# DJjjjhao/FIRA-ICSE

Measured on AMD Instinct MI355X. Metric: training commits/sec (FIRA default config), higher is better.
Workload: dtype f32; 1 GPU; BASELINE configs[1]: FIRA training step (fwd+bwd+Adam, dropout 0.1/0.2), batch 32 commits/GPU, fp32, 650-node graphs (mean nnz 1066/graph), vocab 24650; global_batch=32, parallelism=dp1

## Files before the change

### fira_icse_amd/_lib.py

```python
from __future__ import annotations

import ctypes as C
import os

HERE = os.path.dirname(os.path.abspath(__file__))
LIB_PATH = os.environ.get("FIRA_HIP_LIB") or os.path.join(HERE, "libfira_hip.so")


class FiraError(RuntimeError):
    pass


class Dims(C.Structure):
    _fields_ = [("sou_len", C.c_int32), ("sub_len", C.c_int32), ("ast_len", C.c_int32), ("tar_len", C.c_int32),
                ("d_model", C.c_int32), ("n_head", C.c_int32), ("n_layer", C.c_int32), ("vocab", C.c_int32),
                ("ast_vocab", C.c_int32), ("d_ff", C.c_int32)]


class Batch(C.Structure):
    _fields_ = [("B", C.c_int32), ("nnz", C.c_int32), ("sou", C.c_void_p), ("tar", C.c_void_p), ("mark", C.c_void_p),
                ("ast_change", C.c_void_p), ("tar_label", C.c_void_p), ("sub_token", C.c_void_p),
                ("n_nodes", C.c_int32), ("node_rows", C.c_void_p), ("rowptr", C.c_void_p), ("col", C.c_void_p),
                ("val", C.c_void_p), ("n_code", C.c_int32), ("code_rows", C.c_void_p), ("code_mark", C.c_void_p),
                ("n_mem", C.c_int32), ("mem_rows", C.c_void_p), ("mem_dst", C.c_void_p), ("head_rows", C.c_void_p),
# ... 43 lines not shown
    "fira_linear_x3": (_I, [_P, _I, _I, _P, _I, _P, _P, _P, _I, _I]),
    "fira_linear_dgrad_x3": (_I, [_P, _I, _I, _P, _I, _P, _P, _I, _I, _I]),
    "fira_dgrad_x3_splitk_planes_bytes": (_Z, [_I]),
    "fira_dgrad_x3_splitk": (_I, [_P, _I, _I, _P, _I, _P, _P, _P, _I, _I]),
    "fira_head_logits_x3_scratch_bytes": (_Z, [_I]),
    "fira_head_logits_x3": (_I, [_P, _I, _I, _P, _I, _P, _P, _P, _I, _P]),
    "fira_combination_block_fwd": (_I, [_P, _I, _P, _P, _P, _P, _P, _P, _P, _I, _P, _P, _P, _P, _P, _P, _P, _P, _P, _F, _U64, _U32, _U32, _I]),
    "fira_combination_block_bwd": (_I, [_P, _I, _P, _P, _P, _P, _P, _P, _P, _P, _P, _I, _P, _P, _P, _P, _P, _P, _I, _P, _F, _U64, _U32, _U32, _I]),
    "fira_combination_block_bwd_part_floats": (_I, []),
    "fira_embed_gather_fwd": (_I, [_P, _I, _I, _P, _P, _P, _P, _I, _I]),
    "fira_embed_gather_bwd": (_I, [_P, _I, _I, _P, _P, _P, _I, _I, _I]),
    "fira_combination_fwd": (_I, [_P, _I, _P, _P, _P, _P, _F, _U64, _U32]),
    "fira_combination_bwd": (_I, [_P, _I, _P, _P, _P, _P, _P, _P, _F, _U64, _U32]),
    "fira_add_layernorm_fwd": (_I, [_P, _I, _P, _P, _P, _P, _P, _P, _F, _U64, _U32]),
    "fira_linear_presum_f32": (_I, [_P, _I, _I, _P, _I, _P, _P, _P, _P, _F, _U64, _U32]),
    "fira_ln_linear_f32": (_I, [_P, _I, _I, _P, _I, _P, _P, _P, _I, _I, _P, _P, _P, _P]),
    "fira_ln_bwd_linear_f32": (_I, [_P, _I, _I, _P, _P, _P, _P, _P, _P, _P, _P, _P, _P, _P, _P, _F, _U64, _U32]),
    "fira_linear_layernorm_bf16_fwd": (_I, [_P, _I, _P, _I, _P, _I, _P, _P, _P, _P, _P, _P, _P, _F, _U64, _U32]),
    "fira_add_layernorm_bwd": (_I, [_P, _I, _P, _P, _P, _P, _P, _P, _P, _P, _F, _U64, _U32]),
    "fira_dropout_mask": (_I, [_P, _U64, _U32, _L, _F, _P]),
    "fira_colsum_f32": (_I, [_P, _I, _I, _P, _I, _P]),
    "fira_attention_fwd": (_I, [_P, _I, _I, _I, _I, _P, _I, _P, _I, _P, _I, _P, _I, _I, _P, _I]),
    "fira_attention_bwd": (_I, [_P, _I, _I, _I, _I, _P, _I, _P, _I, _P, _I, _P, _I, _I, _P, _I, _P, _I,
                                _P, _I, _P, _I, _P, _I]),
    "fira_attention_fwd_ex": (_I, [_P, _I, _I, _I, _I, _P, _I, _P, _I, _P, _I, _P, _I, _I, _P, _I, _P, _I, _I, _P]),
    "fira_attention_bwd_ex": (_I, [_P, _I, _I, _I, _I, _P, _I, _P, _I, _P, _I, _P, _I, _I, _P, _I, _P, _I,
                                   _P, _I, _P, _I, _P, _I, _P, _I, _I, _P]),
    "fira_decode_attention": (_I, [_P, _I, _I, _I, _P, _I, _P, _I, _P, _I, _P, _P, _I, _I, _I, _I, _P, _P, _I, _P, _P, _P]),
    "fira_copy_score_fwd": (_I, [_P, _I, _I, _I, _P, _P, _P, _P, _P]),
    "fira_copy_score_bwd": (_I, [_P, _I, _I, _I, _P, _P, _P, _P, _P, _P, _P, _P]),
    "fira_head_loss": (_I, [_P, _I, _I, _I, _I, _P, _P, _I, _P, _P, _P, _P, _P, _P, _P, _I]),
    "fira_adam_step": (_I, [_P, _L, _P, _P, _P, _P, _F, _F, _F, _F, _I, _P]),
    "fira_adam_step_mb": (_I, [_P, _L, _P, _P, _P, _P, _P, _F, _F, _F, _F, _I, _P, _P]),
    "fira_inv_count": (_I, [_P, _P, _P]),
    "fira_adam_step_count": (_I, [_P, _L, _P, _P, _P, _P, _F, _F, _F, _F, _I, _P]),
    "fira_pack_stats": (_I, [_P, _P, _P, _P]),
    "fira_debug_chain": (_I, [_P, _I, _I, _P]),
    "fira_train_fwd_bwd": (_I, [_P, _DP, _BP, _P, _P, _P, _Z, _OP, _P, _P, _P]),
    "fira_train_step": (_I, [_P, _DP, _BP, _P, _P, _P, _Z, _OP, _P, _P, C.POINTER(AdamOpts)]),
    "fira_gemm_wgrad_panel": (_I, [_P, _I, _I, _I, _I, _P, _I, _P, _I, _P, _I, _P, _P, _Z]),
    "fira_ffn_fwd": (_I, [_P, _I, _I] + [_P] * 11 + [_F, _U64, _U32, _I]),
    "fira_ffn_bwd": (_I, [_P, _I, _I] + [_P] * 17 + [_F, _U64, _U32, _I]),
    "fira_head_topk": (_I, [_P, _I, _I, _I, _P, _P, _P, _P, _I, _P, _P, _I]),
    "fira_train_step_rows": (_I, [_P, _DP, _BP, _P, _P, _P, _Z, _OP, _P, _P, C.POINTER(AdamOpts), _P]),
    "fira_adam_rows_sync": (_I, [_P, _DP, _P, C.POINTER(AdamOpts), _P]),
    "fira_adam_rows_catchup": (_I, [_P, _DP, _P, C.POINTER(AdamOpts), _P, _I, _P, _I]),
    "fira_adam_rows_step": (_I, [_P, _DP, _P, _P, C.POINTER(AdamOpts), _P, _P, _P, _I]),
    "fira_train_step_begin_rows": (_I, [_P, _DP, _BP, _P, _P, _P, _Z, _OP, _P, _P, _P, C.POINTER(AdamOpts), _P]),
    "fira_train_step_end_rows": (_I, [_P, _P, C.POINTER(AdamOpts), _P, _P, _P]),
    "fira_grad_sqsum_scratch_bytes": (_Z, []),
    "fira_grad_sqsum": (_I, [_P, _L, _P, _P, _I, _P]),
    "fira_clip_finish": (_I, [_P, _P, _I, _P, _P, _F]),
    "fira_adam_step_clip": (_I, [_P, _L, _P, _P, _P, _P, _F, _F, _F, _F, _I, _P, _P, _P]),
    "fira_adam_rows_step_clip": (_I, [_P, _DP, _P, _P, C.POINTER(AdamOpts), _P, _P, _P, _I, _P]),
    "fira_train_step_clip": (_I, [_P, _DP, _BP, _P, _P, _P, _Z, _OP, _P, _P, C.POINTER(AdamOpts), _P, _F, _P, _P]),
    "fira_train_step_begin": (_I, [_P, _DP, _BP, _P, _P, _P, _Z, _OP, _P, _P, _P]),
    "fira_train_step_end": (_I, [_P, _P, C.POINTER(AdamOpts), _P, _P]),
    "fira_f32_to_bf16": (_I, [_P, _L, _P, _P]),
    "fira_bf16_to_f32": (_I, [_P, _L, _P, _P]),
    "fira_prof_enable": (None, [_I]),
    "fira_prof_report": (_I, [_I, C.POINTER(C.c_double), C.POINTER(C.c_double), C.POINTER(C.c_double), C.POINTER(_L)]),
    "fira_param_groups": (_I, [_DP, C.POINTER(_L), C.POINTER(_L)]),
    "fira_host_node_lists": (_I, [_I, _I, _I, _I, _I] + [_P] * 7 + [_I] + [_P] * 14),
    "fira_host_collate_csr": (_I, [_I, _I, _P, _L, _P, _P, _P, _P, _P, _P, _P]),
    "fira_forward_dev": (_I, [_P, _DP, _BP, _P, _P, _Z, _P, _P, _P, _I]),
    "fira_decode_begin": (_I, [_P, _DP, _BP, _P, _P, _Z, _I]),
# ... 94 lines not shown
```

### fira_icse_amd/csrc/copyhead.hip

```cpp
#include "engine.h"
#include "adam_rows.h"
#include <stdlib.h>
#include "epilogue.h"
#include "decode_row.h"

namespace fira {

constexpr int T_MAX = 32;

__device__ __forceinline__ float tanh_fast(float x) {
    const float e = __expf(2.0f * x);
    return 1.0f - __fdividef(2.0f, 1.0f + e);
}

__global__ __launch_bounds__(256) void copy_score_fwd_kernel(int T, int S, const float* __restrict__ src,
                                                             const float* __restrict__ tgt,
                                                             const float* __restrict__ w,
                                                             const float* __restrict__ bias,
                                                             float* __restrict__ score, int qpk,
                                                             const int32_t* __restrict__ mem_valid, int slots,
                                                             const int32_t* __restrict__ tar_label, int V,
                                                             const int32_t* __restrict__ t_off) {
    __shared__ __attribute__((aligned(16))) float sm_tgt[T_MAX * FIRA_D];
    __shared__ unsigned sm_mask;
// ... 777 lines not shown
}
int head_loss(hipStream_t s, int BT, int T, int V, int S, const int32_t* compact_row, float* logits, int ldl,
              float* score, const int32_t* mem_valid, float* gate_logits, const int32_t* tar_label, float* loss_sum,
              int32_t* n_tok, int32_t* argmax_out, int want_grad, const int32_t* row_bt) {
    ProfScope prof(s, PROF_HEAD, 0.0);
    if (BT <= 0) return 0;
    const bool reg = (V % 2 == 0) && (V / 2 <= 256 * HL_PAIRS) && (ldl % 2 == 0) && ((uintptr_t)logits % 8 == 0);
    if (reg && !argmax_out)
        hipLaunchKernelGGL(head_loss_train_kernel, dim3(BT), dim3(256), 0, s, T, V, S, compact_row, logits, ldl, score,
                           mem_valid, gate_logits, tar_label, loss_sum, n_tok, want_grad, row_bt);
    else if (reg)
        hipLaunchKernelGGL(head_loss_kernel<true>, dim3(BT), dim3(256), 0, s, T, V, S, compact_row, logits, ldl, score,
                           mem_valid, gate_logits, tar_label, loss_sum, n_tok, argmax_out, want_grad, row_bt);
    else
        hipLaunchKernelGGL(head_loss_kernel<false>, dim3(BT), dim3(256), 0, s, T, V, S, compact_row, logits, ldl, score,
                           mem_valid, gate_logits, tar_label, loss_sum, n_tok, argmax_out, want_grad, row_bt);
    FIRA_CHECK_LAUNCH("head_loss");
    return 0;
}
int adam_step(hipStream_t s, int64_t n, float* p, const float* g, float* m, float* v, float lr, float beta1,
              float beta2, float eps, int step, const float* scale_ptr, int scale_is_count) {
    ProfScope prof(s, PROF_ADAM, 0.0);
    if (n <= 0) return 0;
    FIRA_REQUIRE(step >= 1, "adam_step: step must start at 1");
    const double bc1 = 1.0 - pow((double)beta1, step);
    const double bc2 = 1.0 - pow((double)beta2, step);
    const int grid = (int)std::min<int64_t>(cdiv64(n, 256), 256 * 16);
    hipLaunchKernelGGL(adam_kernel, dim3(grid), dim3(256), 0, s, n, p, g, m, v, lr, beta1, beta2, eps, (float)bc1,
                       (float)sqrt(bc2), scale_ptr, scale_is_count);
    FIRA_CHECK_LAUNCH("adam_step");
    return 0;
}
int adam_step_mb(hipStream_t s, int64_t n, float* p, const float* g0, const float* g1, float* m, float* v, float lr,
                 float beta1, float beta2, float eps, int step, const int32_t* n0, const int32_t* n1) {
    ProfScope prof(s, PROF_ADAM, 0.0);
    if (n <= 0) return 0;
    const double bc1 = 1.0 - pow((double)beta1, step);
    const double bc2 = 1.0 - pow((double)beta2, step);
    const int grid = (int)std::min<int64_t>(cdiv64(n, 256), 256 * 16);
    hipLaunchKernelGGL(adam_mb_kernel, dim3(grid), dim3(256), 0, s, n, p, g0, g1, m, v, lr, beta1, beta2, eps, (float)bc1,
                       (float)sqrt(bc2), n0, n1);
    FIRA_CHECK_LAUNCH("adam_step_mb");
    return 0;
}
AdamRowsHist adam_rows_hist(float beta1, float beta2, int end) {
    AdamRowsHist h;
    for (int k = 0; k < ADAM_ROWS_K; ++k) h.bc1[k] = h.bc2s[k] = 1.f;
    for (int j = std::max(1, end - ADAM_ROWS_K + 1); j <= end; ++j) {
        h.bc1[j % ADAM_ROWS_K] = (float)(1.0 - pow((double)beta1, j));
        h.bc2s[j % ADAM_ROWS_K] = (float)sqrt(1.0 - pow((double)beta2, j));
    }
    return h;
}
AdamRowsView adam_rows_view(const AdamRowsTables& tb, int table, float lr, float beta1, float beta2, float eps, int to) {
    AdamRowsView vw;
    if (to < 1) return vw;
    vw.m = tb.m + tb.off[table]; vw.v = tb.v + tb.off[table];
    vw.last = tb.last + (table ? tb.rows[0] : 0);
    vw.to = to; vw.lr = lr; vw.beta1 = beta1; vw.beta2 = beta2; vw.eps = eps; vw.gz = 0.f;
    vw.h = adam_rows_hist(beta1, beta2, to);
    return vw;
}
int adam_rows_step(hipStream_t s, const AdamRowsTables& tb, const float* g, float lr, float beta1, float beta2, float eps,
                   int step, const int32_t* n0, const float* count, int tables) {
    ProfScope prof(s, PROF_ADAM, 0.0);
    FIRA_REQUIRE(step >= 1 && tb.last && (n0 || count), "adam_rows_step: bad argument");
    const int it_lo = (tables & 1) ? 0 : tb.rows[0], it_hi = (tables & 2) ? tb.rows[0] + tb.rows[1] : tb.rows[0];
    const int total = it_hi - it_lo;
    if (total <= 0) return 0;
    const int grid = std::min(cdiv(total, 16), 256 * 8);
    hipLaunchKernelGGL(adam_rows_kernel, dim3(grid), dim3(256), 0, s, tb, g, lr, beta1, beta2, eps, step,
                       adam_rows_hist(beta1, beta2, step), n0, count, step % ADAM_ROWS_K == 0 ? 1 : 0, 0.0f, it_lo, it_hi);
// ... 13 lines not shown
    hipLaunchKernelGGL(adam_rows_catchup_kernel, dim3(grid), dim3(256), 0, s, tb, l, lr, beta1, beta2, eps, to,
                       adam_rows_hist(beta1, beta2, to), 0.0f);
    FIRA_CHECK_LAUNCH("adam_rows_catchup");
    return 0;
}
int inv_count(hipStream_t s, const int32_t* n_tok, float* out) {
    hipLaunchKernelGGL(inv_count_kernel, dim3(1), dim3(1), 0, s, n_tok, out);
    FIRA_CHECK_LAUNCH("inv_count");
    return 0;
}

}

extern "C" {
int fira_copy_score_fwd(void* stream, int B, int T, int S, const float* src, const float* tgt, const float* w,
                        const float* bias, float* score) {
    return fira::copy_score_fwd((hipStream_t)stream, B, T, S, src, tgt, w, bias, score);
}
int fira_copy_score_bwd(void* stream, int B, int T, int S, const float* src, const float* tgt, const float* w,
                        const float* dscore, float* dsrc, float* dtgt, float* dw, float* dbias) {
    return fira::copy_score_bwd((hipStream_t)stream, B, T, S, src, tgt, w, dscore, dsrc, dtgt, dw, dbias);
}
int fira_head_loss(void* stream, int BT, int T, int V, int S, const int32_t* compact_row, float* logits, int ldl,
                   float* score, const int32_t* mem_valid, float* gate_logits, const int32_t* tar_label,
                   float* loss_sum, int32_t* n_tok, int32_t* argmax_out, int want_grad) {
    return fira::head_loss((hipStream_t)stream, BT, T, V, S, compact_row, logits, ldl, score, mem_valid, gate_logits,
                           tar_label, loss_sum, n_tok, argmax_out, want_grad);
}
int fira_adam_step_mb(void* stream, int64_t n, float* p, const float* g0, const float* g1, float* m, float* v, float lr,
                      float beta1, float beta2, float eps, int step, const int32_t* n_tok0, const int32_t* n_tok1) {
    FIRA_REQUIRE(p && g0 && m && v && n_tok0 && step >= 1, "fira_adam_step_mb: bad argument");
    return fira::adam_step_mb((hipStream_t)stream, n, p, g0, g1, m, v, lr, beta1, beta2, eps, step, n_tok0, n_tok1);
}
int fira_inv_count(void* stream, const int32_t* n_tok, float* out) {
    return fira::inv_count((hipStream_t)stream, n_tok, out);
}
int fira_adam_step(void* stream, int64_t n, float* p, const float* g, float* m, float* v, float lr, float beta1,
                   float beta2, float eps, int step, const float* inv_scale_ntok) {
    return fira::adam_step((hipStream_t)stream, n, p, g, m, v, lr, beta1, beta2, eps, step, inv_scale_ntok, 0);
}
int fira_adam_step_count(void* stream, int64_t n, float* p, const float* g, float* m, float* v, float lr, float beta1,
                         float beta2, float eps, int step, const float* count) {
    FIRA_REQUIRE(p && g && m && v && count && step >= 1, "fira_adam_step_count: bad argument");
    return fira::adam_step((hipStream_t)stream, n, p, g, m, v, lr, beta1, beta2, eps, step, count, 1);
}
int fira_pack_stats(void* stream, const float* loss_sum, const int32_t* n_tok, float* out2) {
    FIRA_REQUIRE(loss_sum && n_tok && out2, "fira_pack_stats: null pointer argument");
    hipLaunchKernelGGL(fira::pack_stats_kernel, dim3(1), dim3(1), 0, (hipStream_t)stream, loss_sum, n_tok, out2);
    FIRA_CHECK_LAUNCH("pack_stats");
    return 0;
}
}
```

### fira_icse_amd/csrc/engine.h

```cpp
#pragma once
#include "common.h"
#include <string>
#include <vector>

namespace fira {

int gemm_f32(hipStream_t s, int tA, int tB, int M, int N, int K, const float* A, int lda, const float* B, int ldb,
             float* C, int ldc, const float* bias, int flags, int splitk);
int gemm_f32_ex(hipStream_t s, int tA, int tB, int M, int N, int K, const float* A, int lda, const float* B, int ldb,
                float* C, int ldc, const float* bias, int flags, int splitk, float* colsum,
                const int32_t* c_rows = nullptr, const float* relu_mask = nullptr);
int gemm_bf16_ex(hipStream_t s, int tA, int tB, int M, int N, int K, const float* A, int lda, const float* B, int ldb,
                 float* C, int ldc, const float* bias, int flags, int splitk, float* colsum,
                 const int32_t* c_rows = nullptr, const float* relu_mask = nullptr);
struct ShadowEntry { int64_t offset; int rows, cols, pitch_t; int64_t offset_t; };
constexpr int SHADOW_MAX = 64;
struct ShadowTable {
    int n = 0;
    int64_t wbt_elems = 0;
    int tile_start[SHADOW_MAX + 1] = {0};
    ShadowEntry e[SHADOW_MAX];
};
int weight_shadows(hipStream_t s, const ShadowTable& tab, const float* P, uint16_t* Wb, uint16_t* WbT);
int gemm_bf16_wb_ex(hipStream_t s, int M, int N, int K, const float* A, int lda, const uint16_t* Bb, int ldb, float* C,
// ... 176 lines not shown
                   const float* bias, float* score);
int copy_score_fwd_ex(hipStream_t s, int B, int T, int S, const float* src, const float* tgt, const float* w,
                      const float* bias, float* score, int qpk, const int32_t* mem_valid,
                      const int32_t* tar_label = nullptr, int V = 0,
                      const int32_t* t_off = nullptr);
int copy_score_bwd_ex(hipStream_t s, int B, int T, int S, const float* src, const float* tgt, const float* w,
                      const float* dscore, float* dsrc, float* dtgt, float* dw, float* dbias, const int32_t* mem_valid,
                      float* part = nullptr, const int32_t* t_off = nullptr);
int copy_score_bwd_blocks(int B, int S);
constexpr int COPY_PART_STRIDE = 264;
int decode_dist(hipStream_t s, int R, int V, int S, const float* logits, int ldl, const float* score,
                const int32_t* mem_valid, int qpk, const float* gate_logits, float* dist, int32_t* best_id,
                float* best_p, const float* x = nullptr, const float* wp = nullptr, const float* bp = nullptr);
int inv_count(hipStream_t s, const int32_t* n_tok, float* out);
int sample_dist(hipStream_t s, int R, int n_sample, int V, int S, const float* logits, int ldl, const float* score,
                const int32_t* mem_valid, const float* x, const float* wp, const float* bp, int T, int step,
                const int32_t* key, const uint64_t* seed_dev, float temperature, int top_k, float top_p, float* dist,
                int32_t* best_id, float* best_p);
int score_dist(hipStream_t s, int R, int n_cand, int V, int L, int S, const float* logits, int ldl, const float* score,
               const int32_t* mem_valid, const float* x, const float* wp, const float* bp, const int32_t* target,
               const int32_t* label, const int32_t* sou, const int32_t* sub, float* dist, float* p_word, float* p_entry,
               int32_t* entry, float* copy_share, float* p_label, int32_t* top_id, float* logp_word, float* logp_entry,
               float* logp_label);
int row_topk(hipStream_t s, int R, int V, int k, const float* logits, int ldl, int32_t* ids, float* vals);
int copy_score_bwd(hipStream_t s, int B, int T, int S, const float* src, const float* tgt, const float* w,
                   const float* dscore, float* dsrc, float* dtgt, float* dw, float* dbias);
int head_loss(hipStream_t s, int BT, int T, int V, int S, const int32_t* compact_row, float* logits, int ldl,
              float* score, const int32_t* mem_valid, float* gate_logits, const int32_t* tar_label, float* loss_sum,
              int32_t* n_tok, int32_t* argmax_out, int want_grad,
              const int32_t* row_bt = nullptr);
int adam_step(hipStream_t s, int64_t n, float* p, const float* g, float* m, float* v, float lr, float beta1,
              float beta2, float eps, int step, const float* scale_ptr, int scale_is_count = 0);
int adam_step_mb(hipStream_t s, int64_t n, float* p, const float* g0, const float* g1, float* m, float* v, float lr,
                 float beta1, float beta2, float eps, int step, const int32_t* n0, const int32_t* n1);
constexpr int ADAM_ROWS_K = 32;
struct AdamRowsHist { float bc1[ADAM_ROWS_K], bc2s[ADAM_ROWS_K]; };
struct AdamRowsTables { float *p, *m, *v; int64_t off[2]; int rows[2]; int32_t* last; };
struct AdamRowsView {
    const float *m = nullptr, *v = nullptr;
    const int32_t* last = nullptr;
    int to = 0;
    float lr = 0.f, beta1 = 0.f, beta2 = 0.f, eps = 0.f, gz = 0.f;
    AdamRowsHist h;
};
AdamRowsView adam_rows_view(const AdamRowsTables& tb, int table, float lr, float beta1, float beta2, float eps, int to);
struct AdamRowsLists { int n_lists; int end[4]; int table[4]; const int32_t* ids[4]; };
int adam_rows_step(hipStream_t s, const AdamRowsTables& tb, const float* g, float lr, float beta1, float beta2, float eps,
                   int step, const int32_t* n0, const float* count, int tables = 3);
int adam_rows_catchup(hipStream_t s, const AdamRowsTables& tb, const AdamRowsLists* ls, float lr, float beta1, float beta2,
                      float eps, int to);
AdamRowsHist adam_rows_hist(float beta1, float beta2, int end);
struct ClipClose {
    const int32_t* n_tok;
    const float* count;
    float max_norm;
    int n_slots;
};
size_t grad_sqsum_scratch_bytes();
int grad_sqsum(hipStream_t s, int64_t n, const float* g, fira_clip_state* st, int slot, void* scratch, const ClipClose* fin);
int clip_finish(hipStream_t s, fira_clip_state* st, const ClipClose& fin);
int adam_step_clip(hipStream_t s, int64_t n, float* p, const float* g, float* m, float* v, float lr, float beta1, float beta2,
                   float eps, int step, const int32_t* n0, const float* count, const fira_clip_state* st);
int adam_rows_step_clip(hipStream_t s, const AdamRowsTables& tb, const float* g, float lr, float beta1, float beta2, float eps,
                        int step, const int32_t* n0, const float* count, int tables, const fira_clip_state* st);

struct ParamInfo {
    std::string name;
// ... 25 lines not shown
```

### fira_icse_amd/csrc/engine.hip

```cpp
#include "engine.h"
#include <hip/hip_ext.h>
#include "epilogue.h"
#include <stdlib.h>
#include <map>
#include <mutex>

namespace fira {

static int64_t shadow_wbt_elems(const Layout& L);

struct Arena {
    char* base;
    size_t used = 0;
    explicit Arena(void* b) : base((char*)b) {}
    template <typename T>
    T* get(size_t n) {
        size_t bytes = (n * sizeof(T) + 255) / 256 * 256;
        T* p = base ? (T*)(base + used) : nullptr;
        used += bytes;
        return p;
    }
    float* f(size_t n) { return get<float>(n); }
};

// ... 969 lines not shown
    TRY(linear(s, R, p.V, D, dec_rows, D, c.P + L.wout, c.P + L.bout, p.logits, p.ldl));
    TRY(gemm_any(s, 0, 1, c.Td, D, D, dec, D, c.P + L.wt, D, p.tgt, D, nullptr, 0, 0, nullptr));
    if (c.deferred) TRY(main_wait(s, c.ev_src, __LINE__));
    TRY(copy_score_fwd_ex(s, p.B, p.T, Sm, p.src, p.tgt, c.P + L.wres, c.P + L.bres, p.score, 1, p.mem_valid,
                          argmax_out ? nullptr : c.bt->tar_label, p.V, c.dec_off));
    TRY(linear(s, c.Td, 2, D, dec, D, c.P + L.wp, c.P + L.bp, p.gate, 2));
    TRY(head_loss(s, c.Td, p.T, p.V, Sm, p.compact_row, p.logits, p.ldl, p.score, p.mem_valid, p.gate,
                  c.bt->tar_label, loss_sum, n_tok, argmax_out, want_grad, c.row_bt));
    return 0;
}

static inline int enc_wgrad_every(int n_rows, int n_layers) {
    static const int forced = [] { const char* e = getenv("FIRA_ENC_WGRAD_EVERY"); const int v = e ? atoi(e) : 0; return v >= 1 ? v : 0; }();
    if (forced) return forced;
    return n_rows <= 32768 ? std::max(1, n_layers) : 1;
}

static int group_a_final_stream(hipStream_t s, hipStream_t* out) {
    SideStream& sd = side();
    *out = s;
    if (sd.stream && sd.enabled) {
        TRY(aux_fork(s));
        hipEvent_t e2 = sd.ev();
        if (hipEventRecord(e2, sd.stream) != hipSuccess || hipStreamWaitEvent(sd.aux, e2, 0) != hipSuccess)
            return set_err("group-A mark: weight-gradient stream mark failed");
        *out = sd.aux;
    }
    return 0;
}

struct BwdMid {
    hipEvent_t ev_dmem = nullptr;
    hipEvent_t ev_groupA = nullptr;
};

static int backward_decoder(Ctx& c, int R, const int32_t* rows, hipEvent_t mid_event, BwdMid& mid) {
    Plan& p = *c.pl;
    const Layout& L = *c.L;
    hipStream_t s = c.s;
    const int D = FIRA_D, H = L.d.n_head, KV = p.nl * 2 * D, Sm = p.L + p.S;
    const fira_batch& bt = *c.bt;
    const int Nc = bt.n_nodes, Cc = bt.n_code, Mc = bt.n_mem;
    const float* dec = p.dec[p.nl - 1].x_f;
    float* G = c.G;

    gemm_group_reset();
    gemm_bf16_group_reset();
    gemm_wgrad_panel_reset();
    gemm_wgrad_panel_scratch(p.panel_scratch, p.panel_floats);
    red().reset(p.red_buf, p.red_cap);
    const bool so = side_on();
    hipStream_t ss = so ? side().aux : s;
    hipEvent_t ev_dfc = nullptr;
    if (c.ev_zero) TRY(main_wait(s, c.ev_zero, __LINE__));
    else TRY(zero(s, p.zero_beg, (size_t)((char*)p.zero_end - (char*)p.zero_beg)));
    if (R > 0) {
        if (so) TRY(aux_fork(s));
        if (c.wout_planes) TRY(dgrad_x3_splitk(ss, R, p.V, p.logits, p.ldl, p.WoutTX, p.ddec_c, D, g_dtype == 1));
        else
        TRY(gemm_any(ss, 0, 0, R, D, p.V, p.logits, p.ldl, c.P + L.wout, D, p.ddec_c, D, nullptr, FIRA_GEMM_ACCUM, 0,
                        nullptr));
        if (so) TRY(side_mark(&ev_dfc));
    }
    if (R > 0)
        TRY(linear_wgrad(s, R, p.V, D, p.logits, p.ldl, (c.rows != nullptr && rows == c.rows) ? p.dec_c : dec, D, G + L.wout,
                         G + L.bout, PANEL_VOCAB));
// ... 100 lines not shown
        if (dec_every > 0 && l % dec_every == 0 && side().stream && side().enabled) {
            const int nlay = std::min(dec_every, p.nl - l);
            const size_t o = (size_t)l * 2 * D;
            prof_decoder_tag(-1);
            int rc_w = flush_wgrads_all();
            if (!rc_w)
                rc_w = wgrad_on(side().stream, PANEL_KV, Mc, nlay * 2 * D, D, p.dkv_all + o, p.kvp, p.mem_c, D, G + L.wkv_all + o * D,
                                G + L.bkv_all + o);
            prof_decoder_tag(+1);
            TRY(rc_w);
        }
        float* t = bx; bx = by; by = t;
    }
    TRY(lanes_join(c));
    }
    const float* dy = bx;
    TRY(flush_grouped_wgrads(s));
    {
        hipStream_t es = (side().stream && side().enabled) ? side().stream : s;
        if (c.row_bt) TRY(embed_rows_bwd(es, c.Td, c.row_bt, c.bt->tar, G + L.dec_emb, dy, 0));
        else TRY(embed_gather_bwd(es, p.B, p.T, c.bt->tar, G + L.dec_emb, dy, p.T, 0, 0));
    }
    hipEvent_t& ev_dmem = mid.ev_dmem;
    if (so) {
        TRY(side_mark(&ev_dmem));
    } else {
        TRY(linear_dgrad(s, Mc, KV, D, p.dkv_all, p.kvp, c.P + L.wkv_all, p.dmem_c, D, true));
    }
    if (!(side().stream && side().enabled))
        TRY(linear_wgrad(s, Mc, KV, D, p.dkv_all, p.kvp, p.mem_c, D, G + L.wkv_all, G + L.bkv_all, PANEL_KV));
    else if (dec_every == 0)
        TRY(wgrad_on(side().stream, PANEL_KV, Mc, KV, D, p.dkv_all, p.kvp, p.mem_c, D, G + L.wkv_all, G + L.bkv_all));
    TRY(deferred_reduce(side().stream && side().enabled ? side().stream : s, red().tab));
    hipEvent_t& ev_groupA = mid.ev_groupA;
    if (c.adam && side().stream && side().enabled) {
        ev_groupA = side().ev();
        if (hipEventRecord(ev_groupA, side().stream) != hipSuccess) return set_err("group-A mark failed");
    }
    if (mid_event || c.clip) {
        hipStream_t es = nullptr;
        TRY(group_a_final_stream(s, &es));
        if (mid_event) {
            hipError_t e = hipEventRecord(mid_event, es);
            if (e != hipSuccess) return set_err("hipEventRecord: %s", hipGetErrorString(e));
        }
        if (c.clip) TRY(grad_sqsum(es, L.split, G, c.clip->state, 0, c.clip->scratch, nullptr));
    }
    return 0;
}

static int backward_encoder(Ctx& c, BwdMid& mid) {
    Plan& p = *c.pl;
    const Layout& L = *c.L;
    hipStream_t s = c.s;
    const int D = FIRA_D;
    const fira_batch& bt = *c.bt;
    const int Nc = bt.n_nodes, Cc = bt.n_code, Mc = bt.n_mem;
    float* G = c.G;
    hipEvent_t ev_dmem = mid.ev_dmem, ev_groupA = mid.ev_groupA;
    float* dXn = p.dXa;
    float* other = p.dXb;
    UnfoldTable unfold_tab;
    static const bool unfold_late_off = [] { const char* e = getenv("FIRA_UNFOLD_LATE"); return e && e[0] == '0'; }();
    const bool unfold_late = !unfold_late_off && enc_group_on() && p.nl <= 16;
    const int wgrad_every = unfold_late ? enc_wgrad_every(Nc, p.nl) : 1;
    const float *uf_dW21[16], *uf_W1[16], *uf_W2[16];
    float *uf_dW1[16], *uf_dW2[16];
    int uf_n = 0;
    if (!c.ev_zero) TRY(zero(s, dXn, (size_t)Nc * D * sizeof(float)));
    if (ev_dmem) TRY(main_wait(s, ev_dmem, __LINE__));
    TRY(rows_move(s, 1, Mc, D, dXn, p.dmem_c, nullptr, bt.mem_rows));
    for (int l = p.nl - 1; l >= 0; --l) {
        const EncLayer& w = L.enc[l];
        EncSave& e = p.enc[l];
        EncGrad& g = p.encg[l];
        float* dc21 = p.dc21 + (size_t)l * D;
        bool sums = false;
        const bool room = unfold_tab.n < 16;
        TRY(ln_bwd(s, Nc, dXn, e.s2, e.st2, c.P + w.ln2g, other, g.dY2, G + w.ln2g, G + w.ln2b, c.p_gcn,
                              c.seed, site(l, SITE_GCN), nullptr, room ? p.rsum : nullptr, G + w.fc2b, dc21, &sums));
        if (sums) unfold_tab.e[unfold_tab.n++] = UnfoldEntry{c.P + w.fc2w, c.P + w.fc1b, dc21, G + w.fc2w, G + w.fc1b};
        float* dW21 = p.dW21 + (size_t)l * D * D;
        const bool grouped = enc_group_on();
        bool flushed = false;
        auto unfold = [&]() -> int {
            hipStream_t ws = s;
            if (side().stream && side().enabled) {
                if (!grouped || (!flushed && (!sums || !unfold_late))) TRY(side_fork(s));
                ws = side().stream;
            }
            if (!sums) TRY(colsum(ws, Nc, D, g.dY2, D, dc21, p.rsum));
            if (unfold_late) {
// ... 65 lines not shown
        const bool ax = side_on();
        hipStream_t rs = ax ? side().aux : s;
        if (ax) TRY(aux_fork(s));
        TRY(deferred_reduce(rs, red().tab));
        TRY(gemm_f32_ex(rs, 1, 0, p.nl * D, D, 4, p.dvtab_all, p.nl * D, c.P + L.mark_emb, D, G + L.w2_all, D, nullptr,
                        FIRA_GEMM_ACCUM, 1, G + L.b2_all));
        TRY(gemm_f32_ex(rs, 0, 0, 3, D, p.nl * D, p.dvtab_all + (size_t)p.nl * D, p.nl * D, c.P + L.w2_all, D, G + L.mark_emb + D, D,
                        nullptr, FIRA_GEMM_ACCUM, std::max(2, p.nl), nullptr));
        if (ax) TRY(side_mark(&ev_tail));
    }
    if (bt.emb_item_tok && bt.emb_item_ptr && bt.emb_rows && bt.ast_rows && bt.ast_ids && L.d.ast_vocab <= 128) {
        TRY(embed_grouped_bwd(s, bt.n_emb_items, bt.emb_item_tok, bt.emb_item_ptr, bt.emb_rows, G + L.emb, dXn));
        TRY(embed_list_bwd_small(s, bt.n_ast_items, bt.ast_rows, bt.ast_ids, G + L.ast_emb, dXn, L.d.ast_vocab));
    } else {
        TRY(zero(s, p.H, (size_t)p.NB * D * sizeof(float)));
        TRY(rows_move(s, 1, Nc, D, p.H, dXn, nullptr, bt.node_rows));
        TRY(embed_gather_bwd(s, p.B, p.L, bt.sou, G + L.emb, p.H, p.N, 0, 0));
        TRY(embed_gather_bwd(s, p.B, p.S, bt.sub_token, G + L.emb, p.H, p.N, p.L, 0));
        if (L.d.ast_vocab <= 128)
            TRY(embed_gather_bwd_small(s, p.B, p.A, bt.ast_change, G + L.ast_emb, p.H, p.N, p.L + p.S, 0, L.d.ast_vocab));
        else
            TRY(embed_gather_bwd(s, p.B, p.A, bt.ast_change, G + L.ast_emb, p.H, p.N, p.L + p.S, 0));
    }
    if (c.adam) {
        const fira_adam_opts& ad = *c.adam;
        if (c.adam_a_only) {
            if (c.ev_early) TRY(main_wait(s, c.ev_early, __LINE__));
            const int64_t a0 = c.row_step ? L.dec_emb + (int64_t)L.d.vocab * D : 0;
            if (c.count) TRY(adam_step(s, L.split - a0, c.Pw + a0, G + a0, ad.m + a0, ad.v + a0, ad.lr, ad.beta1, ad.beta2, ad.eps, ad.step, c.count, 1));
            else TRY(adam_step_mb(s, L.split - a0, c.Pw + a0, G + a0, nullptr, ad.m + a0, ad.v + a0, ad.lr, ad.beta1, ad.beta2, ad.eps, ad.step, c.n_tok, nullptr));
            if (c.row_step)
                TRY(adam_rows_step(s, adam_rows_tables(L, c.Pw, ad, c.row_step), G, ad.lr, ad.beta1, ad.beta2, ad.eps, ad.step,
                                   c.count ? nullptr : c.n_tok, c.count, 1));
        } else {
        if (ev_groupA) TRY(main_wait(s, ev_groupA, __LINE__));
        const int64_t a0 = c.row_step ? L.dec_emb + (int64_t)L.d.vocab * D : 0;
        TRY(adam_step_mb(s, L.split - a0, c.Pw + a0, G + a0, nullptr, ad.m + a0, ad.v + a0, ad.lr, ad.beta1, ad.beta2, ad.eps,
                         ad.step, c.n_tok, nullptr));
        }
        if (!c.adam_a_only) adam_b0 = L.mark_emb;
        if (c.row_step && !c.adam_a_only) {
            TRY(adam_rows_step(s, adam_rows_tables(L, c.Pw, ad, c.row_step), G, ad.lr, ad.beta1, ad.beta2, ad.eps, ad.step,
                               c.n_tok, nullptr));
            adam_b0 = L.ast_emb;
        } else
        if (adam_b0 > L.split)
        TRY(adam_step_mb(s, adam_b0 - L.split, c.Pw + L.split, G + L.split, nullptr, ad.m + L.split, ad.v + L.split, ad.lr, ad.beta1,
                         ad.beta2, ad.eps, ad.step, c.n_tok, nullptr));
    }
    if (ev_tail) TRY(main_wait(s, ev_tail, __LINE__));
    if (side().stream && side().enabled) TRY(side_join(s, __LINE__));
    TRY(gcn_bias_unfold_all(s, unfold_tab));
    if (c.adam && !c.adam_a_only) {
        const fira_adam_opts& ad = *c.adam;
        TRY(adam_step_mb(s, L.live - adam_b0, c.Pw + adam_b0, G + adam_b0, nullptr, ad.m + adam_b0, ad.v + adam_b0, ad.lr, ad.beta1,
                         ad.beta2, ad.eps, ad.step, c.n_tok, nullptr));
    }
    if (c.clip) {
        const ClipStep& cl = *c.clip;
        const fira_adam_opts& ad = *cl.adam;
        const ClipClose fin{c.n_tok, nullptr, cl.max_norm, 2};
        TRY(grad_sqsum(s, L.live - L.split, G + L.split, cl.state, 1, cl.scratch, &fin));
        auto dense = [&](int64_t lo, int64_t hi) {
            return adam_step_clip(s, hi - lo, c.Pw + lo, G + lo, ad.m + lo, ad.v + lo, ad.lr, ad.beta1, ad.beta2, ad.eps, ad.step,
                                  c.n_tok, nullptr, cl.state);
        };
        if (c.row_step) {
            const int64_t tab = (int64_t)L.d.vocab * D;
            TRY(adam_rows_step_clip(s, adam_rows_tables(L, c.Pw, ad, c.row_step), G, ad.lr, ad.beta1, ad.beta2, ad.eps, ad.step,
                                    c.n_tok, nullptr, 3, cl.state));
            const int64_t t0 = std::min(L.dec_emb, L.emb), t1 = std::max(L.dec_emb, L.emb);
            TRY(dense(0, t0));
            TRY(dense(t0 + tab, t1));
            TRY(dense(t1 + tab, L.live));
// ... 623 lines not shown
```

### include/fira_hip.h

```cpp
#ifndef FIRA_HIP_H
#define FIRA_HIP_H

#include <stddef.h>
#include <stdint.h>

#ifdef __cplusplus
extern "C" {
#endif

#define FIRA_ABI_VERSION 10

typedef struct fira_dims {
    int32_t sou_len;
    int32_t sub_len;
    int32_t ast_len;
    int32_t tar_len;
    int32_t d_model;
    int32_t n_head;
    int32_t n_layer;
    int32_t vocab;
    int32_t ast_vocab;
    int32_t d_ff;
} fira_dims;

// ... 158 lines not shown
                       int causal, int q_pos0, const float* O, int ldo, const float* dO, int lddo,
                       float* dQ, int lddq, float* dK, int lddk, float* dV, int lddv);
int fira_attention_fwd_ex(void* stream, int B, int H, int Tq, int Tk, const float* Q, int ldq,
                          const float* K, int ldk, const float* V, int ldv, const int32_t* key_valid,
                          int causal, int q_pos0, float* O, int ldo, const int32_t* q_off, int self_kv, int dtype,
                          const int32_t* k_off);
int fira_attention_bwd_ex(void* stream, int B, int H, int Tq, int Tk, const float* Q, int ldq,
                          const float* K, int ldk, const float* V, int ldv, const int32_t* key_valid,
                          int causal, int q_pos0, const float* O, int ldo, const float* dO, int lddo,
                          float* dQ, int lddq, float* dK, int lddk, float* dV, int lddv,
                          const int32_t* q_off, int self_kv, int dtype, const int32_t* k_off);

int fira_decode_attention(void* stream, int BR, int H, int Tk, const float* Q, int ldq, const float* K, int ldk,
                          const float* V, int ldv, const int32_t* key_valid, float* O, int ldo, int kb, int kvb, int qpk,
                          const float* Knew, const float* Vnew, int ldn, float* Kc_out, float* Vc_out,
                          const int32_t* k_off);

int fira_copy_score_fwd(void* stream, int B, int T, int S, const float* src, const float* tgt,
                        const float* w, const float* bias, float* score);
int fira_copy_score_bwd(void* stream, int B, int T, int S, const float* src, const float* tgt,
                        const float* w, const float* dscore, float* dsrc , float* dtgt ,
                        float* dw , float* dbias );

int fira_head_loss(void* stream, int BT, int T, int V, int S, const int32_t* compact_row,
                   float* logits, int ldl, float* score , const int32_t* mem_valid ,
                   float* gate_logits , const int32_t* tar_label ,
                   float* loss_sum, int32_t* n_tok, int32_t* argmax_out, int want_grad);

int fira_adam_step(void* stream, int64_t n, float* p, const float* g, float* m, float* v,
                   float lr, float beta1, float beta2, float eps, int step, const float* inv_scale_ntok);
int fira_adam_step_mb(void* stream, int64_t n, float* p, const float* g0, const float* g1, float* m, float* v,
                      float lr, float beta1, float beta2, float eps, int step, const int32_t* n_tok0,
                      const int32_t* n_tok1);
int fira_adam_step_count(void* stream, int64_t n, float* p, const float* g, float* m, float* v,
                         float lr, float beta1, float beta2, float eps, int step, const float* count);
int fira_pack_stats(void* stream, const float* loss_sum, const int32_t* n_tok, float* out2);
int fira_inv_count(void* stream, const int32_t* n_tok, float* out);

int fira_debug_chain(void* stream, int n, int mode, float* scratch);


int fira_train_fwd_bwd(void* stream, const fira_dims* d, const fira_batch* batch, const float* params,
                       float* grads, void* workspace, size_t workspace_bytes, const fira_train_opts* opts,
                       float* loss_sum, int32_t* n_tok, void* mid_event);

int fira_gemm_wgrad_panel(void* stream, int dtype, int M, int N, int K, const float* A, int lda, const float* B, int ldb,
                          float* C, int ldc, float* colsum, float* scratch, size_t scratch_floats);

int fira_ffn_fwd(void* stream, int M, int F, const float* x, const float* w1, const float* b1, const float* w2, const float* b2,
                 const float* gamma, const float* beta, float* h, float* sum, float* y, float* stats, float dropout,
                 uint64_t seed, uint32_t site, int dtype);
int fira_ffn_bwd(void* stream, int M, int F, const float* dy, const float* x, const float* h, const float* sum,
                 const float* stats, const float* w1, const float* w2, const float* gamma, float* dx, float* dyf_ws,
                 float* dh_ws, float* dw1, float* db1, float* dw2, float* db2, float* dgamma, float* dbeta, float dropout,
                 uint64_t seed, uint32_t site, int dtype);
int fira_head_topk(void* stream, int R, int V, int k, const float* x, const float* wout, const float* bout, float* logits_ws,
                   int ldl, int32_t* ids, float* vals, int dtype);

size_t fira_head_logits_x3_scratch_bytes(int R);
int fira_head_logits_x3(void* stream, int R, int V, const float* x, int ldx, const float* W, const float* bias, float* logits,
                        int ldl, void* scratch);


typedef struct fira_adam_opts {
    float   lr, beta1, beta2, eps;
    int32_t step;
// ... 118 lines not shown
```

Baseline: 13350 commits/s.

## Issue group-A Adam update early on the side stream, capped grid

Moves the Adam update for the decoder parameter range [a0, split) out of the encoder backward and enqueues it on the group-A final stream as soon as the decoder gradients are reduced, when clipping is off. The update can then overlap with the encoder backward on the main stream. Its grid is capped at a smaller block count so it leaves compute units free for the concurrent work. The group-A event is now only recorded in the row-step case and waited on before the row Adam step. This adds cross-stream ordering risk and a longer tail for the smaller grid.

```diff
diff --git a/fira_icse_amd/_lib.py b/fira_icse_amd/_lib.py
--- a/fira_icse_amd/_lib.py
+++ b/fira_icse_amd/_lib.py
@@ -99,6 +99,8 @@
     "fira_head_loss": (_I, [_P, _I, _I, _I, _I, _P, _P, _I, _P, _P, _P, _P, _P, _P, _P, _I]),
     "fira_adam_step": (_I, [_P, _L, _P, _P, _P, _P, _F, _F, _F, _F, _I, _P]),
     "fira_adam_step_mb": (_I, [_P, _L, _P, _P, _P, _P, _P, _F, _F, _F, _F, _I, _P, _P]),
+    "fira_adam_step_mb_grid": (_I, [_P, _L, _P, _P, _P, _P, _P, _F, _F, _F, _F, _I, _P, _P, _I]),
+    "fira_adam_early_blocks": (_I, []),
     "fira_inv_count": (_I, [_P, _P, _P]),
     "fira_adam_step_count": (_I, [_P, _L, _P, _P, _P, _P, _F, _F, _F, _F, _I, _P]),
     "fira_pack_stats": (_I, [_P, _P, _P, _P]),
diff --git a/fira_icse_amd/csrc/copyhead.hip b/fira_icse_amd/csrc/copyhead.hip
--- a/fira_icse_amd/csrc/copyhead.hip
+++ b/fira_icse_amd/csrc/copyhead.hip
@@ -833,12 +833,13 @@
     return 0;
 }
 int adam_step_mb(hipStream_t s, int64_t n, float* p, const float* g0, const float* g1, float* m, float* v, float lr,
-                 float beta1, float beta2, float eps, int step, const int32_t* n0, const int32_t* n1) {
+                 float beta1, float beta2, float eps, int step, const int32_t* n0, const int32_t* n1, int max_blocks) {
     ProfScope prof(s, PROF_ADAM, 0.0);
     if (n <= 0) return 0;
+    FIRA_REQUIRE(max_blocks >= 1, "adam_step_mb: max_blocks=%d", max_blocks);
     const double bc1 = 1.0 - pow((double)beta1, step);
     const double bc2 = 1.0 - pow((double)beta2, step);
-    const int grid = (int)std::min<int64_t>(cdiv64(n, 256), 256 * 16);
+    const int grid = (int)std::min<int64_t>(cdiv64(n, 256), max_blocks);
     hipLaunchKernelGGL(adam_mb_kernel, dim3(grid), dim3(256), 0, s, n, p, g0, g1, m, v, lr, beta1, beta2, eps, (float)bc1,
                        (float)sqrt(bc2), n0, n1);
     FIRA_CHECK_LAUNCH("adam_step_mb");
@@ -918,6 +919,13 @@
     FIRA_REQUIRE(p && g0 && m && v && n_tok0 && step >= 1, "fira_adam_step_mb: bad argument");
     return fira::adam_step_mb((hipStream_t)stream, n, p, g0, g1, m, v, lr, beta1, beta2, eps, step, n_tok0, n_tok1);
 }
+int fira_adam_step_mb_grid(void* stream, int64_t n, float* p, const float* g0, const float* g1, float* m, float* v, float lr,
+                           float beta1, float beta2, float eps, int step, const int32_t* n_tok0, const int32_t* n_tok1,
+                           int max_blocks) {
+    FIRA_REQUIRE(p && g0 && m && v && n_tok0 && step >= 1 && max_blocks >= 1, "fira_adam_step_mb_grid: bad argument");
+    return fira::adam_step_mb((hipStream_t)stream, n, p, g0, g1, m, v, lr, beta1, beta2, eps, step, n_tok0, n_tok1, max_blocks);
+}
+int fira_adam_early_blocks(void) { return fira::ADAM_EARLY_BLOCKS; }
 int fira_inv_count(void* stream, const int32_t* n_tok, float* out) {
     return fira::inv_count((hipStream_t)stream, n_tok, out);
 }
diff --git a/fira_icse_amd/csrc/engine.h b/fira_icse_amd/csrc/engine.h
--- a/fira_icse_amd/csrc/engine.h
+++ b/fira_icse_amd/csrc/engine.h
@@ -232,7 +232,9 @@
 int adam_step(hipStream_t s, int64_t n, float* p, const float* g, float* m, float* v, float lr, float beta1,
               float beta2, float eps, int step, const float* scale_ptr, int scale_is_count = 0);
 int adam_step_mb(hipStream_t s, int64_t n, float* p, const float* g0, const float* g1, float* m, float* v, float lr,
-                 float beta1, float beta2, float eps, int step, const int32_t* n0, const int32_t* n1);
+                 float beta1, float beta2, float eps, int step, const int32_t* n0, const int32_t* n1,
+                 int max_blocks = 256 * 16);
+constexpr int ADAM_EARLY_BLOCKS = 512;
 constexpr int ADAM_ROWS_K = 32;
 struct AdamRowsHist { float bc1[ADAM_ROWS_K], bc2s[ADAM_ROWS_K]; };
 struct AdamRowsTables { float *p, *m, *v; int64_t off[2]; int rows[2]; int32_t* last; };
diff --git a/fira_icse_amd/csrc/engine.hip b/fira_icse_amd/csrc/engine.hip
--- a/fira_icse_amd/csrc/engine.hip
+++ b/fira_icse_amd/csrc/engine.hip
@@ -1025,6 +1025,7 @@
 struct BwdMid {
     hipEvent_t ev_dmem = nullptr;
     hipEvent_t ev_groupA = nullptr;
+    bool adam_a_early = false;
 };
 
 static int backward_decoder(Ctx& c, int R, const int32_t* rows, hipEvent_t mid_event, BwdMid& mid) {
@@ -1191,12 +1192,12 @@
     else if (dec_every == 0)
         TRY(wgrad_on(side().stream, PANEL_KV, Mc, KV, D, p.dkv_all, p.kvp, p.mem_c, D, G + L.wkv_all, G + L.bkv_all));
     TRY(deferred_reduce(side().stream && side().enabled ? side().stream : s, red().tab));
-    hipEvent_t& ev_groupA = mid.ev_groupA;
-    if (c.adam && side().stream && side().enabled) {
-        ev_groupA = side().ev();
-        if (hipEventRecord(ev_groupA, side().stream) != hipSuccess) return set_err("group-A mark failed");
-    }
-    if (mid_event || c.clip) {
+    const bool adam_a_early = c.adam && !c.adam_a_only && !c.clip;
+    if (adam_a_early && c.row_step && side().stream && side().enabled) {
+        mid.ev_groupA = side().ev();
+        if (hipEventRecord(mid.ev_groupA, side().stream) != hipSuccess) return set_err("group-A mark failed");
+    }
+    if (mid_event || c.clip || adam_a_early) {
         hipStream_t es = nullptr;
         TRY(group_a_final_stream(s, &es));
         if (mid_event) {
@@ -1204,6 +1205,13 @@
             if (e != hipSuccess) return set_err("hipEventRecord: %s", hipGetErrorString(e));
         }
         if (c.clip) TRY(grad_sqsum(es, L.split, G, c.clip->state, 0, c.clip->scratch, nullptr));
+        if (adam_a_early) {
+            const fira_adam_opts& ad = *c.adam;
+            const int64_t a0 = c.row_step ? L.dec_emb + (int64_t)L.d.vocab * D : 0;
+            TRY(adam_step_mb(es, L.split - a0, c.Pw + a0, G + a0, nullptr, ad.m + a0, ad.v + a0, ad.lr, ad.beta1, ad.beta2, ad.eps,
+                             ad.step, c.n_tok, nullptr, ADAM_EARLY_BLOCKS));
+            mid.adam_a_early = true;
+        }
     }
     return 0;
 }
@@ -1216,7 +1224,7 @@
     const fira_batch& bt = *c.bt;
     const int Nc = bt.n_nodes, Cc = bt.n_code, Mc = bt.n_mem;
     float* G = c.G;
-    hipEvent_t ev_dmem = mid.ev_dmem, ev_groupA = mid.ev_groupA;
+    hipEvent_t ev_dmem = mid.ev_dmem;
     float* dXn = p.dXa;
     float* other = p.dXb;
     UnfoldTable unfold_tab;
@@ -1348,14 +1356,10 @@
             if (c.row_step)
                 TRY(adam_rows_step(s, adam_rows_tables(L, c.Pw, ad, c.row_step), G, ad.lr, ad.beta1, ad.beta2, ad.eps, ad.step,
                                    c.count ? nullptr : c.n_tok, c.count, 1));
-        } else {
-        if (ev_groupA) TRY(main_wait(s, ev_groupA, __LINE__));
-        const int64_t a0 = c.row_step ? L.dec_emb + (int64_t)L.d.vocab * D : 0;
-        TRY(adam_step_mb(s, L.split - a0, c.Pw + a0, G + a0, nullptr, ad.m + a0, ad.v + a0, ad.lr, ad.beta1, ad.beta2, ad.eps,
-                         ad.step, c.n_tok, nullptr));
-        }
+        } else if (!mid.adam_a_early) return set_err("backward_encoder: the update of [0, split) was not enqueued");
         if (!c.adam_a_only) adam_b0 = L.mark_emb;
         if (c.row_step && !c.adam_a_only) {
+            if (mid.ev_groupA) TRY(main_wait(s, mid.ev_groupA, __LINE__));
             TRY(adam_rows_step(s, adam_rows_tables(L, c.Pw, ad, c.row_step), G, ad.lr, ad.beta1, ad.beta2, ad.eps, ad.step,
                                c.n_tok, nullptr));
             adam_b0 = L.ast_emb;
diff --git a/include/fira_hip.h b/include/fira_hip.h
--- a/include/fira_hip.h
+++ b/include/fira_hip.h
@@ -214,6 +214,10 @@
 int fira_adam_step_mb(void* stream, int64_t n, float* p, const float* g0, const float* g1, float* m, float* v,
                       float lr, float beta1, float beta2, float eps, int step, const int32_t* n_tok0,
                       const int32_t* n_tok1);
+int fira_adam_step_mb_grid(void* stream, int64_t n, float* p, const float* g0, const float* g1, float* m, float* v,
+                           float lr, float beta1, float beta2, float eps, int step, const int32_t* n_tok0,
+                           const int32_t* n_tok1, int max_blocks);
+int fira_adam_early_blocks(void);
 int fira_adam_step_count(void* stream, int64_t n, float* p, const float* g, float* m, float* v,
                          float lr, float beta1, float beta2, float eps, int step, const float* count);
 int fira_pack_stats(void* stream, const float* loss_sum, const int32_t* n_tok, float* out2);
```

Measured after the change: 13100 commits/s. -1.8%, worse.
